# bupt-cist/vqa-playground-pytorch

Hardware: AMD Instinct MI355X
Metric: VQA samples/sec (fwd+bwd), CoR2 batch 512, 36x2048 regions (higher is better)
Workload: dtype f32

## Files before the change

vqa_playground_pytorch_amd/csrc/bilinear_rt.hip:

```cpp
#include <cstdlib>

#include "bilinear_folded.hpp"
#include "gemm_f32_rt.hpp"

namespace vqa {
namespace {

struct FoldRtArgs {
  const float* x;
  const float* w[2];
  const float* bias[2];
  const float* h2;
  float* out;
  int ldx, ldw, ldh2, ldo;
  int B, N, K, NO;
  int tiles_o;
};

constexpr int kNB = 3;

template <bool FWD, int S, int IB, int R, int FG = 1>
__global__ __launch_bounds__(rt::kThreads, 1) void bilinear_fold_rt_kernel(FoldRtArgs p) {
  using rt::f32x4;
  const int lane = threadIdx.x & 63, r = lane & 15, g = lane >> 4;
  const int wave = __builtin_amdgcn_readfirstlane(threadIdx.x >> 6);
  const int tile = xcd_remap(blockIdx.x, gridDim.x);
  const int b0 = (tile / p.tiles_o) * S;
  const int o0 = (tile % p.tiles_o) * (64 * IB) + wave * (16 * IB);
  const int B = p.B, N = p.N, K = p.K, NO = p.NO;
  if (o0 >= NO) return;

  rt::rsrc_t Wb[R];
#pragma unroll
  for (int rk = 0; rk < R; ++rk) Wb[rk] = rt::make_rsrc(p.w[rk], ((size_t)(NO - 1) * p.ldw + K) * 4);
  const rt::rsrc_t Xb = rt::make_rsrc(p.x, ((size_t)(B * N - 1) * p.ldx + K) * 4);
  const rt::rsrc_t Hb = rt::make_rsrc(p.h2, (size_t)B * R * p.ldh2 * 4);
  uint32_t offW[IB], offX[S][kNB], offH[S];
#pragma unroll
  for (int i = 0; i < IB; ++i) offW[i] = ((uint32_t)min(o0 + 16 * i + r, NO - 1) * (uint32_t)p.ldw + 4u * g) * 4u;
#pragma unroll
  for (int s = 0; s < S; ++s) {
    const int b = min(b0 + s, B - 1);
#pragma unroll
    for (int j = 0; j < kNB; ++j) offX[s][j] = ((uint32_t)(b * N + min(16 * j + r, N - 1)) * (uint32_t)p.ldx + 4u * g) * 4u;
    offH[s] = (uint32_t)(b * R) * (uint32_t)p.ldh2 * 4u;
  }
  float hrow[FWD ? S : 1][R][FWD ? IB : 1];
  if constexpr (FWD) {
#pragma unroll
    for (int s = 0; s < S; ++s)
#pragma unroll
      for (int rk = 0; rk < R; ++rk)
#pragma unroll
        for (int i = 0; i < IB; ++i)
          hrow[s][rk][i] = rt::ldg4(Hb, offH[s] + (uint32_t)(rk * p.ldh2 + min(o0 + 16 * i + r, NO - 1)) * 4u, 0u);
  }

  f32x4 acc[S][IB][kNB];
#pragma unroll
  for (int s = 0; s < S; ++s)
#pragma unroll
    for (int i = 0; i < IB; ++i)
#pragma unroll
      for (int j = 0; j < kNB; ++j) acc[s][i][j] = f32x4{0.f, 0.f, 0.f, 0.f};

  struct Frag {
    f32x4 w[R][IB];
    f32x4 x[S][kNB];
    f32x4 hk[FWD ? 1 : S][R];
  };
  auto load = [&](Frag& f, int c) {
    const uint32_t so = (uint32_t)c * 64u;
#pragma unroll
    for (int rk = 0; rk < R; ++rk)
#pragma unroll
      for (int i = 0; i < IB; ++i) f.w[rk][i] = rt::ldg16(Wb[rk], offW[i], so);
#pragma unroll
    for (int s = 0; s < S; ++s) {
#pragma unroll
      for (int j = 0; j < kNB; ++j) f.x[s][j] = rt::ldg16(Xb, offX[s][j], so);
      if constexpr (!FWD) {
#pragma unroll
        for (int rk = 0; rk < R; ++rk) f.hk[s][rk] = rt::ldg16(Hb, offH[s] + (uint32_t)(rk * p.ldh2) * 4u + 16u * g, so);
      }
    }
  };
  auto fold = [&](const Frag& f, int s, int i) -> f32x4 {
    typedef float f32x2 __attribute__((ext_vector_type(2)));
    f32x4 we;
    if constexpr (FWD) {
      const f32x2 h0 = f32x2{hrow[s][0][i], hrow[s][0][i]};
      f32x2 lo = f32x2{f.w[0][i][0], f.w[0][i][1]} * h0, hi = f32x2{f.w[0][i][2], f.w[0][i][3]} * h0;
      if constexpr (R == 2) {
        const f32x2 h1 = f32x2{hrow[s][1][i], hrow[s][1][i]};
        lo = __builtin_elementwise_fma(f32x2{f.w[1][i][0], f.w[1][i][1]}, h1, lo);
        hi = __builtin_elementwise_fma(f32x2{f.w[1][i][2], f.w[1][i][3]}, h1, hi);
      }
      we = f32x4{lo[0], lo[1], hi[0], hi[1]};
    } else {
      f32x2 lo = f32x2{f.w[0][i][0], f.w[0][i][1]} * f32x2{f.hk[s][0][0], f.hk[s][0][1]};
      f32x2 hi = f32x2{f.w[0][i][2], f.w[0][i][3]} * f32x2{f.hk[s][0][2], f.hk[s][0][3]};
      if constexpr (R == 2) {
        lo = __builtin_elementwise_fma(f32x2{f.w[1][i][0], f.w[1][i][1]}, f32x2{f.hk[s][1][0], f.hk[s][1][1]}, lo);
        hi = __builtin_elementwise_fma(f32x2{f.w[1][i][2], f.w[1][i][3]}, f32x2{f.hk[s][1][2], f.hk[s][1][3]}, hi);
      }
      we = f32x4{lo[0], lo[1], hi[0], hi[1]};
    }
    return we;
  };
  auto compute = [&](const Frag& f, auto pin, auto nloads) {
    constexpr bool PIN = decltype(pin)::value;
    constexpr int NL = decltype(nloads)::value;
    constexpr int NQ = S * IB;
    constexpr int NV = R == 2 ? 4 : 2;
    f32x4 we[FG], wn[FG];
#pragma unroll
    for (int t = 0; t < FG; ++t) we[t] = fold(f, min(t, NQ - 1) / IB, min(t, NQ - 1) % IB);
    if constexpr (PIN) __builtin_amdgcn_sched_group_barrier(0x002, NV * FG, 0);
    int issued = 0;
#pragma unroll
    for (int q0 = 0; q0 < NQ; q0 += FG) {
#pragma unroll
      for (int t = 0; t < FG; ++t) wn[t] = we[t];
      if (q0 + FG < NQ) {
#pragma unroll
        for (int t = 0; t < FG; ++t)
          if (q0 + FG + t < NQ) {
            wn[t] = fold(f, (q0 + FG + t) / IB, (q0 + FG + t) % IB);
            if constexpr (PIN) __builtin_amdgcn_sched_group_barrier(0x002, NV, 0);
          }
      }
#pragma unroll
      for (int t = 0; t < FG; ++t) {
        const int q = q0 + t;
        if (q >= NQ) break;
        const int s = q / IB, i = q % IB;
#pragma unroll
        for (int kb = 0; kb < 4; ++kb)
#pragma unroll
          for (int j = 0; j < kNB; ++j) {
            acc[s][i][j] = __builtin_amdgcn_mfma_f32_16x16x4f32(we[t][kb], f.x[s][j][kb], acc[s][i][j], 0, 0, 0);
            if constexpr (PIN) {
              __builtin_amdgcn_sched_group_barrier(0x008, 1, 0);
              const int m = q * 4 * kNB + kb * kNB + j;
              if (issued < NL && (m + 1) * NL / (NQ * 4 * kNB) > issued) {
                __builtin_amdgcn_sched_group_barrier(0x020, 1, 0);
                ++issued;
              }
            }
          }
      }
#pragma unroll
      for (int t = 0; t < FG; ++t) we[t] = wn[t];
    }
  };
  auto step = [&](Frag& fn, int cn, const Frag& f) {
    constexpr int NL = R * IB + S * kNB + (FWD ? 0 : S * R);
    load(fn, cn);
    compute(f, std::true_type{}, std::integral_constant<int, NL>{});
    __builtin_amdgcn_sched_barrier(0);
  };

  const int nfull = K >> 4;
  const int c_pairs = nfull & ~1;
  {
    Frag f0, f1;
    if (c_pairs > 0) {
      load(f0, 0);
      __builtin_amdgcn_sched_barrier(0);
      for (int c = 0; c < c_pairs; c += 2) {
        step(f1, c + 1, f0);
        step(f0, min(c + 2, c_pairs - 1), f1);
      }
    }
    if (c_pairs < nfull) {
      load(f0, c_pairs);
      compute(f0, std::false_type{}, std::integral_constant<int, 0>{});
    }
  }
  if ((K & 15) != 0 || FWD) {
    Frag f;
#pragma unroll
    for (int kb = 0; kb < 4; ++kb) {
      const int k = 16 * nfull + 4 * g + kb;
      const bool in = k < K;
      const uint32_t kc = (uint32_t)min(k, K - 1);
#pragma unroll
      for (int rk = 0; rk < R; ++rk)
#pragma unroll
        for (int i = 0; i < IB; ++i) {
          float v = rt::ldg4(Wb[rk], offW[i] - 16u * g + kc * 4u, 0u);
          v = in ? v : 0.f;
          if constexpr (FWD) {
            if (k == K) v = p.bias[rk][min(o0 + 16 * i + r, NO - 1)];
          }
          f.w[rk][i][kb] = v;
        }
#pragma unroll
      for (int s = 0; s < S; ++s) {
#pragma unroll
        for (int j = 0; j < kNB; ++j) {
          float v = rt::ldg4(Xb, offX[s][j] - 16u * g + kc * 4u, 0u);
          v = in ? v : 0.f;
          if constexpr (FWD) {
            if (k == K) v = 1.f;
          }
          f.x[s][j][kb] = v;
        }
        if constexpr (!FWD) {
#pragma unroll
          for (int rk = 0; rk < R; ++rk) {
            const float v = rt::ldg4(Hb, offH[s] + (uint32_t)(rk * p.ldh2) * 4u + kc * 4u, 0u);
            f.hk[s][rk][kb] = in ? v : 0.f;
          }
        }
      }
    }
    compute(f, std::false_type{}, std::integral_constant<int, 0>{});
  }

#pragma unroll
  for (int s = 0; s < S; ++s) {
    const int b = b0 + s;
    if (b >= B) break;
#pragma unroll
    for (int j = 0; j < kNB; ++j) {
      const int n = 16 * j + r;
      if (n >= N) continue;
      float* __restrict__ row = p.out + (size_t)(b * N + n) * p.ldo;
#pragma unroll
      for (int i = 0; i < IB; ++i) {
        const int o = o0 + 16 * i + 4 * g;
        if (o + 3 < NO) {
          *reinterpret_cast<f32x4*>(row + o) = acc[s][i][j];
        } else {
#pragma unroll
          for (int t = 0; t < 4; ++t)
            if (o + t < NO) row[o + t] = acc[s][i][j][t];
        }
      }
    }
  }
}

template <bool FWD>
int launch(const FoldRtArgs& a0, int R, hipStream_t s) {
  FoldRtArgs a = a0;
  constexpr int S = FWD ? 4 : 2, IB = FWD ? 4 : 5;
  a.tiles_o = (a.NO + 64 * IB - 1) / (64 * IB);
  const dim3 grid((unsigned)(((a.B + S - 1) / S) * a.tiles_o));
  const char* fg_opt = vqa::option("VQA_K4_FG");
  const int fg = fg_opt != nullptr ? std::atoi(fg_opt) : (FWD ? 4 : 2);
  if (R == 1)
    VQA_LAUNCH((bilinear_fold_rt_kernel<FWD, S, IB, 1>), grid, dim3(rt::kThreads), 0, s, a);
  else if (fg == 2)
    VQA_LAUNCH((bilinear_fold_rt_kernel<FWD, S, IB, 2, 2>), grid, dim3(rt::kThreads), 0, s, a);
  else if (fg == 4)
    VQA_LAUNCH((bilinear_fold_rt_kernel<FWD, S, IB, 2, 4>), grid, dim3(rt::kThreads), 0, s, a);
  else
    VQA_LAUNCH((bilinear_fold_rt_kernel<FWD, S, IB, 2>), grid, dim3(rt::kThreads), 0, s, a);
  return check_launch(FWD ? "lowrank_bilinear_fusion_folded_fwd (register-tile)" : "lowrank_bilinear_fusion_folded_bwd (dx, register-tile)");
}

}

bool fold_rt_supported(int B, int N, int K, int NO, int R, int ldx, int ldw, int ldo) {
  const bool off = vqa::option_is("VQA_K4_RT", '0');
  return !off && R >= 1 && R <= 2 && N > 16 && N <= 48 && B >= 256 && K >= 32 && NO >= 64 && ldx % 2 == 0 && ldw % 2 == 0 &&
         ldo % 2 == 0 && (size_t)B * N * (size_t)(ldx > ldo ? ldx : ldo) * 4 < (1ull << 32) && (size_t)NO * ldw * 4 < (1ull << 32);
}

int fold_rt_forward(const float* x, int ldx, const float* const* w1, const float* const* b1, const float* h2, float* out, int B,
                    int N, int L, int H, int R, hipStream_t s) {
  FoldRtArgs a{};
  a.x = x;
  for (int r = 0; r < R; ++r) {
    a.w[r] = w1[r];
    a.bias[r] = b1[r];
  }
  a.h2 = h2;
  a.out = out;
  a.ldx = ldx;
  a.ldw = L;
  a.ldh2 = H;
  a.ldo = H;
  a.B = B;
  a.N = N;
  a.K = L;
  a.NO = H;
  return launch<true>(a, R, s);
}

int fold_rt_data_gradient(const float* g, const float* const* w1t, const float* h2, float* d_x, int B, int N, int L, int H, int R,
                          hipStream_t s) {
  FoldRtArgs a{};
  a.x = g;
  for (int r = 0; r < R; ++r) a.w[r] = w1t[r];
  a.h2 = h2;
  a.out = d_x;
  a.ldx = H;
  a.ldw = H;
  a.ldh2 = H;
  a.ldo = L;
  a.B = B;
  a.N = N;
  a.K = H;
  a.NO = L;
  return launch<false>(a, R, s);
}

}
```

Measured before the change: 260,600.

## Use 4x4x1 MFMA for the 4-region tail block when N is 33-36

When the region count N is between 33 and 36, the third 16-row region block holds at most 4 valid rows. That block now uses the 4x4x1 f32 MFMA instead of 16x16x4, cutting wasted padded MFMA work. Partial sums across the four 4x4 blocks are reduced with ds_bpermute lane exchanges before the store. The cost is extra cross-lane shuffles, a different output store pattern, and a second kernel body instantiation selected at runtime.

```diff
diff --git a/vqa_playground_pytorch_amd/csrc/bilinear_rt.hip b/vqa_playground_pytorch_amd/csrc/bilinear_rt.hip
--- a/vqa_playground_pytorch_amd/csrc/bilinear_rt.hip
+++ b/vqa_playground_pytorch_amd/csrc/bilinear_rt.hip
@@ -19,8 +19,13 @@
 
 constexpr int kNB = 3;
 
-template <bool FWD, int S, int IB, int R, int FG = 1>
-__global__ __launch_bounds__(rt::kThreads, 1) void bilinear_fold_rt_kernel(FoldRtArgs p) {
+template <int X>
+__device__ __forceinline__ float lane_xor(float v, int lane) {
+  return __builtin_bit_cast(float, __builtin_amdgcn_ds_bpermute((lane ^ X) << 2, __builtin_bit_cast(int, v)));
+}
+
+template <bool FWD, int S, int IB, int R, int FG, bool T4>
+__device__ __forceinline__ void bilinear_fold_rt_body(const FoldRtArgs& p) {
   using rt::f32x4;
   const int lane = threadIdx.x & 63, r = lane & 15, g = lane >> 4;
   const int wave = __builtin_amdgcn_readfirstlane(threadIdx.x >> 6);
@@ -42,7 +47,10 @@
   for (int s = 0; s < S; ++s) {
     const int b = min(b0 + s, B - 1);
 #pragma unroll
-    for (int j = 0; j < kNB; ++j) offX[s][j] = ((uint32_t)(b * N + min(16 * j + r, N - 1)) * (uint32_t)p.ldx + 4u * g) * 4u;
+    for (int j = 0; j < kNB; ++j) {
+      const int n = T4 && j == 2 ? 32 + (r & 3) : 16 * j + r;
+      offX[s][j] = ((uint32_t)(b * N + min(n, N - 1)) * (uint32_t)p.ldx + 4u * g) * 4u;
+    }
     offH[s] = (uint32_t)(b * R) * (uint32_t)p.ldh2 * 4u;
   }
   float hrow[FWD ? S : 1][R][FWD ? IB : 1];
@@ -138,8 +146,16 @@
 #pragma unroll
         for (int kb = 0; kb < 4; ++kb)
 #pragma unroll
-          for (int j = 0; j < kNB; ++j) {
-            acc[s][i][j] = __builtin_amdgcn_mfma_f32_16x16x4f32(we[t][kb], f.x[s][j][kb], acc[s][i][j], 0, 0, 0);
+          for (int jj = 0; jj < kNB; ++jj) {
+            const int j = T4 ? (jj + 2) % kNB : jj;
+            if constexpr (T4) {
+              if (j == 2)
+                acc[s][i][j] = __builtin_amdgcn_mfma_f32_4x4x1f32(we[t][kb], f.x[s][j][kb], acc[s][i][j], 0, 0, 0);
+              else
+                acc[s][i][j] = __builtin_amdgcn_mfma_f32_16x16x4f32(we[t][kb], f.x[s][j][kb], acc[s][i][j], 0, 0, 0);
+            } else {
+              acc[s][i][j] = __builtin_amdgcn_mfma_f32_16x16x4f32(we[t][kb], f.x[s][j][kb], acc[s][i][j], 0, 0, 0);
+            }
             if constexpr (PIN) {
               __builtin_amdgcn_sched_group_barrier(0x008, 1, 0);
               const int m = q * 4 * kNB + kb * kNB + j;
@@ -223,8 +239,31 @@
   for (int s = 0; s < S; ++s) {
     const int b = b0 + s;
     if (b >= B) break;
-#pragma unroll
-    for (int j = 0; j < kNB; ++j) {
+    if constexpr (T4) {
+      const int n = 32 + (r & 3);
+      float* __restrict__ row = p.out + (size_t)(b * N + min(n, N - 1)) * p.ldo;
+#pragma unroll
+      for (int i = 0; i < IB; ++i) {
+        f32x4 v = acc[s][i][2];
+#pragma unroll
+        for (int t = 0; t < 4; ++t) {
+          v[t] += lane_xor<16>(v[t], lane);
+          v[t] += lane_xor<32>(v[t], lane);
+        }
+        const int o = o0 + 16 * i + 4 * (r >> 2);
+        if (n < N && g == (i & 3)) {
+          if (o + 3 < NO) {
+            *reinterpret_cast<f32x4*>(row + o) = v;
+          } else {
+#pragma unroll
+            for (int t = 0; t < 4; ++t)
+              if (o + t < NO) row[o + t] = v[t];
+          }
+        }
+      }
+    }
+#pragma unroll
+    for (int j = 0; j < (T4 ? 2 : kNB); ++j) {
       const int n = 16 * j + r;
       if (n >= N) continue;
       float* __restrict__ row = p.out + (size_t)(b * N + n) * p.ldo;
@@ -241,6 +280,14 @@
       }
     }
   }
+}
+
+template <bool FWD, int S, int IB, int R, int FG = 1>
+__global__ __launch_bounds__(rt::kThreads, 1) void bilinear_fold_rt_kernel(FoldRtArgs p) {
+  if (p.N > 32 && p.N <= 36)
+    bilinear_fold_rt_body<FWD, S, IB, R, FG, true>(p);
+  else
+    bilinear_fold_rt_body<FWD, S, IB, R, FG, false>(p);
 }
 
 template <bool FWD>
```

Result: slower. 257,800 (-1.1%).
